# eddyxzc/lpopc

Measured on AMD Instinct MI355X. Metric: eval_g+eval_jac_g calls/sec, 4-phase 4096-LGR-pt problem, higher is better.
Workload: dtype f64

## Files before the change

lpopc_amd/csrc/rpm_abi.cpp:

```cpp
#include <cmath>
#include <cstdio>
#include <cstring>
#include <vector>
#include <new>
#include <string>

#include <atomic>

#include "rpm_engine.hpp"
#include "rpm_pin.h"

static thread_local std::string g_create_error;

using rpm::Engine;

#define RPM_GUARD_BEGIN try {
#define RPM_GUARD_END(eng)                                   \
  }                                                          \
  catch (const std::exception& ex) {                         \
    (eng).err = std::string("internal error: ") + ex.what(); \
    return RPM_E_INVALID;                                    \
  }                                                          \
  catch (...) {                                              \
    (eng).err = "internal error";                            \
// ... 660 lines not shown
      e.role_looped = value == 1 || (value == -1 && total / 64 >= 512);
      rpm::build_tiles(e, e.role_looped ? 64 : 16);
    }
  } else
    return fail(e, RPM_E_INVALID, "unknown option");
  rpm::host_new_x(e);
  rpm::dev_forget_persistent(e);
  return RPM_OK;
}
int rpm_get_option(rpm_engine* h, const char* key, int* value) {
  if (!h || !key || !value) return RPM_E_INVALID;
  Engine& e = h->e;
  const std::string k(key);
  if (k == "fuse_pair") *value = e.opt_fuse_pair;
  else if (k == "check_finite") *value = e.opt_check_finite;
  else if (k == "dx_mode") *value = e.opt_dx_mode;
  else if (k == "tile_nodes") *value = e.tile_nodes;
  else if (k == "n_tiles") *value = int(e.tiles.size());
  else if (k == "role_loop") *value = e.role_looped ? 1 : 0;
  else if (k == "pipeline") *value = e.opt_pipeline;
  else if (k == "mesh_err_tile") *value = e.opt_mesh_err_tile;
  else if (k == "carry_tile") *value = e.opt_carry_tile;
  else if (k == "carry_lds_bytes") *value = e.opt_carry_lds;
  else if (k == "carry_groups") *value = rpm::carry_group_count(e);
  else if (k == "extract_tile") *value = e.opt_extract_tile;
  else if (k == "extract_lds_bytes") *value = e.opt_extract_lds;
  else if (k == "extract_groups") *value = rpm::extract_group_count(e);
  else if (k == "stage_roles") *value = e.opt_stage_roles;
  else if (k == "const_once") *value = e.opt_const_once;
  else if (k == "instance_align") *value = e.opt_instance_align;
  else if (k == "delta_values") *value = e.opt_delta_values;
  else if (k == "ipm_nested") *value = e.opt_ipm_nested;
  else if (k == "ipm_nested_group") *value = e.opt_ipm_nested_group;
  else if (k == "ipm_local_border") *value = e.opt_ipm_local_border;
  else if (k == "zero_copy") *value = e.opt_zero_copy;
  else if (k == "persistent_values") *value = e.opt_persistent_values;
  else if (k == "pin_host") *value = e.opt_pin_host;
  else if (k == "pin_registered") *value = int(rpm::dev_pin_counter(RPM_PIN_REGISTERED));
  else if (k == "pin_register_failures") *value = int(rpm::dev_pin_counter(RPM_PIN_REGISTER_FAILURES));
  else if (k == "pin_unregistered") *value = int(rpm::dev_pin_counter(RPM_PIN_UNREGISTERED));
  else if (k == "pin_unregister_failures") *value = int(rpm::dev_pin_counter(RPM_PIN_UNREGISTER_FAILURES));
  else if (k == "pin_overlap_refused") *value = int(rpm::dev_pin_counter(RPM_PIN_OVERLAP_REFUSED));
  else if (k == "pin_shared") *value = int(rpm::dev_pin_counter(RPM_PIN_SHARED));
  else if (k == "pin_merged") *value = int(rpm::dev_pin_counter(RPM_PIN_MERGED));
  else if (k == "pin_evicted") *value = int(rpm::dev_pin_counter(RPM_PIN_EVICTED));
  else if (k == "pin_live") *value = int(rpm::dev_pin_counter(RPM_PIN_LIVE));
  else if (k == "pin_live_kb") *value = int(rpm::dev_pin_counter(RPM_PIN_LIVE_BYTES) / 1024);
  else if (k == "pin_held") *value = rpm::dev_pin_held(e);
  else if (k == "delta_sent_runs") return rpm::host_delta_sent_runs(e, value);
  else if (k == "delta_total_runs") *value = e.last_delta_total;
  else if (k == "stride_g") *value = int(e.stride_g());
  else if (k == "stride_values") *value = int(e.stride_values());
  else if (k == "pipeline_active") *value = rpm::dev_pipeline_active(e);
  else if (k == "hess_tile_nodes") *value = rpm::dev_hess_tile_nodes(e);
  else return fail(e, RPM_E_INVALID, "unknown option");
  return RPM_OK;
}

int rpm_get_phase_sizes(rpm_engine* h, int phase, int* n_nodes, int* d_nnz, int* doff_nnz) {
  if (!h) return RPM_E_INVALID;
  Engine& e = h->e;
  if (phase < 0 || phase >= e.P) return fail(e, RPM_E_INVALID, "The phase index is out of rang");
  if (n_nodes) *n_nodes = e.ph[phase].N;
  if (d_nnz) *d_nnz = int(e.ph[phase].d_v.size());
  if (doff_nnz) *doff_nnz = int(e.ph[phase].off_v.size());
  return RPM_OK;
}
int rpm_get_phase_tables(rpm_engine* h, int phase, double* points, double* weights, int* d_rows, int* d_cols,
                         double* d_vals, double* diag_vals, int* doff_rows, int* doff_cols, double* doff_vals) {
  if (!h) return RPM_E_INVALID;
  Engine& e = h->e;
  if (phase < 0 || phase >= e.P) return fail(e, RPM_E_INVALID, "The phase index is out of rang");
  const rpm::PhaseHost& p = e.ph[phase];
  auto cp = [](auto* dst, const auto& v) {
    if (dst && !v.empty()) std::memcpy(dst, v.data(), v.size() * sizeof(v[0]));
  };
  cp(points, p.points);
  cp(weights, p.weights);
  cp(d_rows, p.d_i);
  cp(d_cols, p.d_j);
  cp(d_vals, p.d_v);
  cp(diag_vals, p.diag_v);
  cp(doff_rows, p.off_i);
  cp(doff_cols, p.off_j);
  cp(doff_vals, p.off_v);
  return RPM_OK;
}

int rpm_shard_segments(rpm_engine* h, int which, int rank, rpm_segment* seg, int* n_seg, int* packed_len) {
  if (!h) return RPM_E_INVALID;
  Engine& e = h->e;
  RPM_GUARD_BEGIN
  if (which < 0 || which > 1 || rank < 0 || rank >= e.shard_world) return fail(e, RPM_E_INVALID, "shard_segments: bad argument");
  int plen = 0;
  std::vector<rpm_segment> s = rpm::shard_segments(e, which, rank, &plen);
  if (seg) {
    if (!n_seg || *n_seg < int(s.size())) return fail(e, RPM_E_INVALID, "shard_segments: segment buffer too small");
    std::memcpy(seg, s.data(), s.size() * sizeof(rpm_segment));
  }
  if (n_seg) *n_seg = int(s.size());
  if (packed_len) *packed_len = plen;
  return RPM_OK;
  RPM_GUARD_END(e)
}
int rpm_shard_pack_dev(rpm_engine* h, int which, const double* d_full, double* d_packed, void* stream) {
  if (!h) return RPM_E_INVALID;
// ... 35 lines not shown
```

lpopc_amd/csrc/rpm_engine.hpp:

```cpp
#pragma once
#include <cstddef>
#include <string>
#include <utility>
#include <vector>

#include "../../include/rpm_hip.h"

namespace rpm {

struct PhaseDev {
  int N, nx, nu, nc, ne;
  int nq;
  int phase_num;
  int x_state0;
  int x_control0;
  int x_t0;
  int g0;
  int v_nl0;
  int v_evt0;
  int node0;
  int doff_base;
  int off_nnz;
  int const_cum;
  int tile0, ntiles;
// ... 182 lines not shown
             std::string* why);
  int smooth_enough(int ip, int first_row, int n, const std::vector<double>& tau, const double* state, int ld, int nx) const;
  bool exponent(int ip, double m0, double mf, int N, double e_k, double* q) const;
};
void lagrange_rows(const double* src, int m, const double* dst, int nq, double* H, double* S, int* hit);

void build_mesh_err_tables(const PhaseHost& p, MeshErrTables& t);
bool ph_refine(const PhaseHost& p, const double* rel, double tol, int nmin, int nmax, std::vector<double>& mesh,
               std::vector<int>& nodes, std::vector<double>& interval_error);
int dev_solution_error(Engine& e, int phase, const double* x, double* rel_err);
void solution_error_batch_sizes(const Engine& e, int* n_intervals_total, long long* rel_doubles_total);
constexpr double mesh_err_max(double a, double v) { return (v > a || v != v) ? v : a; }
int dev_solution_error_batch(Engine& e, const double* d_x, const int* d_mask, double* d_interval_error, double* d_rel_err_max,
                             double* d_rel_err, int* d_nonfinite, void* stream);
int host_solution_error_batch(Engine& e, const double* x, const int* mask, double* interval_error, double* rel_err_max,
                              double* rel_err, int* nonfinite);

int carry_check(Engine& from, const Engine& to, const void* x_from, const void* x_to);
int carry_group_count(const Engine& from);
int dev_carry_batch(Engine& from, Engine& to, const double* d_x_from, double* d_x_to, int* d_nonfinite, void* stream);
int host_carry_batch(Engine& from, Engine& to, const double* x_from, double* x_to, int* nonfinite);

void nlp2op_batch_layout(const Engine& e, int phase, long long field_offset[8], long long* block_doubles);
int extract_check(Engine& e);
int extract_group_count(const Engine& e);
int dev_nlp2op_batch(Engine& e, const double* d_x, const double* d_lambda, double* d_out, int* d_nonfinite, void* stream);
int host_nlp2op_batch(Engine& e, const double* x, const double* lambda, double* out, int* nonfinite);

std::vector<rpm_segment> shard_segments(const Engine& e, int which, int rank, int* packed_len);
int dev_shard_copy(Engine& e, int which, bool pack, const double* src, int stride, double* dst, void* stream);
long long shard_slot_len(const Engine& e);
int dev_shard_pack_all(Engine& e, const double* d_g, const double* d_values, double* d_slot, void* stream);
int dev_shard_unpack_all(Engine& e, const double* d_gathered, double* d_g, double* d_values, int skip_own, void* stream);

struct ProblemDims { int nx, nu, nc, ne_max, nlink_max, nconst; bool has_analytic; int nq; };
bool problem_dims(int problem_id, ProblemDims* out);

int device_init(Engine& e, int device_id);
void device_destroy(Engine& e);
int dev_eval_cons(Engine& e, const double* d_x, double* d_g, double* d_values, int flags, void* stream);
int dev_eval_obj(Engine& e, const double* d_x, double* d_obj, double* d_grad, void* stream, bool host_chk = false);
bool dev_cons_is_one_role(const Engine& e);
int host_eval_f(Engine& e, const double* x, int new_x, double* obj);
int host_eval_grad_f(Engine& e, const double* x, int new_x, double* grad);
int host_eval_g(Engine& e, const double* x, int new_x, double* g);
void host_new_x(Engine& e);
int host_eval_jac_values(Engine& e, const double* x, int new_x, double* values);
int host_eval_pair(Engine& e, const double* x, double* g, double* values);
struct ConsCall { bool want_g, want_v, cached, delta, launched_jac; };
int host_cons_begin(Engine& e, const double* x, int new_x, double* g, double* values, ConsCall* c);
int host_cons_end(Engine& e, double* g, double* values, const ConsCall& c, const char* who);
int host_delta_sent_runs(Engine& e, int* sent);
int dev_pipeline_active(const Engine& e);
int dev_upload_x(Engine& e, const double* x);
int dev_upload(Engine& e, double* dev, const double* host, size_t count, int slot);
int dev_download(Engine& e, double* host, const double* dev, size_t count, int slot);
int dev_sync(Engine& e);
int dev_update_instance_constants(Engine& e);
double* dev_buf(Engine& e, int which);
bool& dev_cache_valid(Engine& e);
void dev_forget_persistent(Engine& e);
void* dev_stream(Engine& e);
int dev_nonfinite(Engine& e, const double* dev, size_t count);
int dev_nonfinite_enqueue(Engine& e, const double* a, size_t na, const double* b, size_t nb);
int dev_flag_value(Engine& e, int slot);
long dev_pin_counter(int which);
int dev_pin_held(const Engine& e);
void* dev_pin_host(Engine& e, const void* ptr, size_t bytes);
void dev_pin_release_all(Engine& e);

}

struct rpm_engine {
  rpm::Engine e;
};
```

lpopc_amd/csrc/rpm_tile_kernels.hip:

```cpp
#include "rpm_device_internal.hpp"

namespace rpm {


template <class Prob, bool WG, bool WJ, bool AN, bool WAVE = false>
__device__ void endpoint_block(const KParams& K, const TaskDev task, const double* __restrict__ x,
                               double* __restrict__ g, double* __restrict__ vals, double* lds, int inst) {
  constexpr int NX = Prob::NX, NQ = prob_nq<Prob>::value, NQs = NQ > 0 ? NQ : 1;
  bool bad_g = false, bad_j = false;
  constexpr int NE = Prob::NE_MAX > 0 ? Prob::NE_MAX : 1;
  constexpr int NL = Prob::NLINK_MAX > 0 ? Prob::NLINK_MAX : 1;
  static_assert(!WAVE || 2 * NX + 3 + 2 * NQ <= 64, "endpoint perturbations must fit one wave");
  const int tid = WAVE ? int(threadIdx.x & 63) : int(threadIdx.x);
  const int nthr = WAVE ? 64 : int(blockDim.x);
  const double* c = K.consts + size_t(inst) * K.consts_stride;
  if (task.type == 0) {
    for (int r = tid; r < K.P + K.L; r += nthr) {
      if (WG) {
        double acc = 0.0;
        acc += K.alin_v[2 * r] * x[K.alin_j[2 * r]];
        acc += K.alin_v[2 * r + 1] * x[K.alin_j[2 * r + 1]];
        g[K.m_nl + r] = acc;
        chk_note(bad_g, acc);
      }
// ... 508 lines not shown
#pragma unroll
          for (int o = 0; o < NO; ++o) {
            double v0, vf;
            if (o < NX) {
              const double fb = Fb[o * T + kk];
              const double dt = J[o] * (tf - t0) / 2.0;
              v0 = fb * (0.5) - a0 * dt;
              vf = -fb * (0.5) + af * dt;
            } else {
              v0 = a0 * J[o];
              vf = af * J[o];
            }
            vb[size_t(o * NB + NX + NU) * N] = v0;
            vb[size_t(o * NB + NX + NU + 1) * N] = vf;
          }
        }
      }
    }
  }
  RPM_TRC(4);
  if (WJ && !K.skip_const) {
    const double* __restrict__ src = K.doff_vals + tl.c_src0;
    double* __restrict__ dst = vals + tl.c_dst0;
    const int lead = int((reinterpret_cast<size_t>(dst) >> 3) & 15);
    for (int q = tid - lead; q < tl.c_cnt; q += NTHR) {
      if (q >= 0) {
        const double dv = src[q];
#pragma unroll
        for (int i = 0; i < NX; ++i) dst[size_t(i) * tl.c_stride + q] = dv;
      }
    }
  }
#ifdef RPM_DIAG
  RPM_TRC(5);
  if (K.trace) {
    __builtin_amdgcn_s_waitcnt(0);
    RPM_TRC(6);
    if (threadIdx.x == 0) {
      unsigned hw;
      asm volatile("s_getreg_b32 %0, hwreg(HW_REG_HW_ID)" : "=s"(hw));
      unsigned xcc;
      asm volatile("s_getreg_b32 %0, hwreg(HW_REG_XCC_ID)" : "=s"(xcc));
      K.trace[(size_t(blockIdx.y) * gridDim.x + blockIdx.x) * 8 + 7] = (static_cast<unsigned long long>(xcc) << 32) | hw;
    }
  }
#endif
}

constexpr int PL_CMAX = 1280, PL_REC = 32;
static_assert(sizeof(TileDev) / sizeof(int) < PL_REC, "tile record plus the instance index must fit the staged record");
static_assert(sizeof(TileDev) % 8 == 0, "the tile record is copied as doubles");

struct PlLds {
  int rec, next, tt, X, U, D, tau, diag, nodes, cv, stage;
  int Fb, ready, DXs, half;
  __host__ __device__ constexpr PlLds(int nx, int nu, int nc, int nq, int max_span, int max_drow, int max_cshare, bool with_jac,
                                      bool dxm)
      : rec(0), next(PL_REC / 2), tt(PL_REC), X(tt + 2 + ((nq + 1) & ~1)), U(X + nx * max_span), D(U + nu * 64),
        tau(D + max_drow), diag(tau + 64), nodes(diag + 64), cv(nodes + 2 * 64), stage(cv + (with_jac ? max_cshare : 0)),
        Fb(2 * stage), ready(Fb + (nx + nc) * 64), DXs(ready + 2), half(DXs + (dxm ? nx * 64 : 0)) {}
};
constexpr bool pl_lds_pinned(int nx, int nu, int nc, int nq, int span, int drow, int cshare, bool wj, bool dxm) {
  const PlLds L(nx, nu, nc, nq, span, drow, cshare, wj, dxm);
  const int nqe = (nq + 1) & ~1;
  return L.rec == 0 && L.next == L.rec + PL_REC / 2 && L.tt == L.next + PL_REC / 2 && L.X == L.tt + 2 + nqe &&
         L.U == L.X + nx * span && L.D == L.U + nu * 64 && L.tau == L.D + drow && L.diag == L.tau + 64 &&
         L.nodes == L.diag + 64 && L.cv == L.nodes + 2 * 64 && L.stage == L.cv + (wj ? cshare : 0) && L.Fb == 2 * L.stage &&
         L.ready == L.Fb + (nx + nc) * 64 && L.DXs == L.ready + 2 && L.half == L.DXs + (dxm ? nx * 64 : 0) &&
         L.stage == PL_REC + 2 + nqe + nx * span + nu * 64 + drow + 4 * 64 + (wj ? cshare : 0) &&
         L.half == 2 * L.stage + (nx + nc) * 64 + 2 + (dxm ? nx * 64 : 0);
}
static_assert(pl_lds_pinned(LaunchProblem::NX, LaunchProblem::NU, LaunchProblem::NC, 0, 73, 64 * 9, 1024, true, false) &&
                  pl_lds_pinned(LaunchProblem::NX, LaunchProblem::NU, LaunchProblem::NC, 1, 80, 64 * 17, 1280, true, true) &&
                  pl_lds_pinned(QuadrotorProblem::NX, QuadrotorProblem::NU, QuadrotorProblem::NC, 0, 65, 64 * 65, 640, false, true),
              "PlLds: an array overlaps its neighbour or a size changed");
typedef double d2u __attribute__((ext_vector_type(2), aligned(8)));
#define RPM_GPTR(p) ((const __attribute__((address_space(1))) void*)(p))
#define RPM_LPTR(p) ((__attribute__((address_space(3))) void*)(p))
template <int NPART>
__device__ __forceinline__ void pl_dma_run(const double* gsrc, double* ldst, int len, int lane, int part) {
  const int pairs = len >> 1;
#pragma unroll 1
  for (int ch = part; ch * 64 < pairs; ch += NPART)
    if (ch * 64 + lane < pairs)
      __builtin_amdgcn_global_load_lds(RPM_GPTR(gsrc + ch * 128 + 2 * lane), RPM_LPTR(ldst + ch * 128), 16, 0, 0);
  if ((len & 1) && part == 0 && lane < 2)
    __builtin_amdgcn_global_load_lds(RPM_GPTR(reinterpret_cast<const int*>(gsrc + len - 1) + lane),
                                     RPM_LPTR(ldst + len - 1), 4, 0, 0);
}


template <int NX, int NPART>
__device__ __forceinline__ void pl_const_stores(const double* cur, const double* cv_src, int inst_word, double* __restrict__ vall,
                                                long long sv, int lane, int part) {
  constexpr int CCH = (PL_CMAX / 128 + NPART - 1) / NPART;
  const int* rec = reinterpret_cast<const int*>(cur);
  const int c_dst0 = RPM_REC(rec, c_dst0);
  const int inst = __builtin_amdgcn_readfirstlane(rec[inst_word]);
  const int c_cnt = RPM_REC(rec, c_cnt);
  const int c_stride = RPM_REC(rec, c_stride);
  double* __restrict__ cdst = vall + size_t(inst) * sv + c_dst0;
  const int head = min(int((16 - ((reinterpret_cast<size_t>(cdst) >> 3) & 15)) & 15), c_cnt);
  d2u cv[CCH];
#pragma unroll
  for (int ch = 0; ch < CCH; ++ch) {
    const int q = max(min(head + (NPART * ch + part) * 128 + 2 * lane, c_cnt - 2), 0);
    cv[ch].x = cv_src[q];
    cv[ch].y = cv_src[q + 1];
  }
  const bool odd_tail = ((c_cnt - head) & 1) != 0;
  const int edge = lane < head ? lane : (lane == head && odd_tail ? c_cnt - 1 : -1);
  const double cedge = cv_src[max(edge, 0)];
#pragma unroll
  for (int ch = 0; ch < CCH; ++ch) {
    const int q = head + (NPART * ch + part) * 128 + 2 * lane;
    if (q + 1 < c_cnt) {
#pragma unroll
      for (int i = 0; i < NX; ++i) __builtin_nontemporal_store(cv[ch], reinterpret_cast<d2u*>(cdst + size_t(i) * c_stride + q));
    }
  }
  if (part == 0 && edge >= 0) {
#pragma unroll
    for (int i = 0; i < NX; ++i) cdst[size_t(i) * c_stride + edge] = cedge;
  }
}

constexpr int pl_role_groups(int R) { return (R + (R + 11) / 12 - 1) / ((R + 11) / 12); }

struct PlShape { int NH, RG, NDMA; };
constexpr PlShape pl_shape(int R) { return R <= 12 ? PlShape{2, 4, 2} : PlShape{1, pl_role_groups(R), 2}; }

template <class Prob, int NH, int RG, int NDMA, bool WG, bool WJ, bool AN, bool DXM = false, bool STG = false>
__global__ __launch_bounds__(NH * 64 * (RG + NDMA), 1) void rpm_tile_pl_kernel(
    const KParams K, int n_inst, const double* __restrict__ xall, double* __restrict__ gall,
    double* __restrict__ vall) {
  constexpr int T = 64;
  constexpr int HT = 64 * (RG + NDMA);
  constexpr int NX = Prob::NX, NU = Prob::NU, NC = Prob::NC, NQ = prob_nq<Prob>::value;
  constexpr int NXs = NX > 0 ? NX : 1, NUs = NU + NQ > 0 ? NU + NQ : 1;
  constexpr int NO = NX + NC, NV = NX + NU + 1 + NQ, NB = NX + NU + 2 + NQ;
  constexpr int R = WJ ? NV + 1 : (NX > 0 ? NX : 1);
  constexpr int NCs = NC > 0 ? NC : 1;
  constexpr int NTHR = T * RG;
  constexpr int NREC = int(sizeof(TileDev) / sizeof(int));
  extern __shared__ double lds_all[];
  const int half = NH > 1 ? __builtin_amdgcn_readfirstlane(int(threadIdx.x) / HT) : 0;
  const int tid = int(threadIdx.x) - half * HT;
  const int nb = int(gridDim.x), wg = xcd_place(int(blockIdx.x), nb);
  const int G = NH * nb, w = NH * wg + half;
  const int nt = K.n_my_tiles;
  const int W = nt * n_inst;
  const int n_iter = w < W ? (W - w + G - 1) / G : 0;
  const int n_iter_wg = (W - NH * wg + G - 1) / G;
  const PlLds L(NX, NU, NC, NQ, K.max_span, K.max_drow, K.max_cshare, WJ, DXM);
  const int S_TT = L.tt, S_X = L.X, S_U = L.U, S_D = L.D, S_TAU = L.tau, S_DG = L.diag, S_ND = L.nodes, S_CV = L.cv, S_SIZE = L.stage;
  double* lds = lds_all + half * L.half;
  double *Fb = lds + L.Fb, *DXs = lds + L.DXs;
  int* fb_ready = reinterpret_cast<int*>(lds + L.ready);
  int* dx_ready = fb_ready + 1;
#ifdef RPM_DIAG
#define RPM_PTRC(j, slot)                                                           \
  if (K.trace && (threadIdx.x & 63) == 0 && (j) < 2) K.trace[size_t(w) * 64 + (j)*32 + (slot)] = wall_clock64()
#define RPM_PEDGE(slot) \
  if (K.trace && (threadIdx.x & 63) == 0) K.trace[size_t(w) * 64 + (slot)] = wall_clock64()
#define RPM_PEDGE_MAX(slot) \
  if (K.trace && (threadIdx.x & 63) == 0) atomicMax(K.trace + size_t(w) * 64 + (slot), (unsigned long long)wall_clock64())
#else
#define RPM_PTRC(j, slot)
#define RPM_PEDGE(slot)
#define RPM_PEDGE_MAX(slot)
#endif
  if (tid == 0) { RPM_PTRC(0, 31); }

  struct TileRuns { int k0, cnt, span0, span_len, drow0, drow_len, N, x_state0, x_control0, x_t0, node0, c_src0, c_cnt; };
  auto runs_of = [&](auto p) {
    return TileRuns{RPM_REC(p, k0), RPM_REC(p, cnt), RPM_REC(p, span0), RPM_REC(p, span_len), RPM_REC(p, drow0),
                    RPM_REC(p, drow_len), RPM_REC(p, N), RPM_REC(p, x_state0), RPM_REC(p, x_control0), RPM_REC(p, x_t0),
                    RPM_REC(p, node0), RPM_REC(p, c_src0), RPM_REC(p, c_cnt)};
  };
  auto stage = [&](auto np_c, int part, int lane, int item, double* buf, const TileRuns tl) {
    constexpr int NP = decltype(np_c)::value;
    const int inst = item / nt, tidx = item - inst * nt;
    const double* __restrict__ x = xall + size_t(inst) * K.n;
    int rot = 0;
    auto run = [&](const double* gsrc, double* ldst, int len) {
      pl_dma_run<NP>(gsrc, ldst, len, lane, (part + NP - (rot++ % NP)) % NP);
    };
    if (part == 0 && lane == 0) reinterpret_cast<int*>(buf + L.rec)[NREC] = inst;
    run(reinterpret_cast<const double*>(K.tiles + tidx), buf + L.rec, NREC / 2);
    if (item + G < W) {
      const int item2 = item + G, inst2 = item2 / nt;
      run(reinterpret_cast<const double*>(K.tiles + (item2 - inst2 * nt)), buf + L.next, NREC / 2);
    }
    run(x + tl.x_t0, buf + S_TT, 2 + NQ);
#pragma unroll
    for (int i = 0; i < NX; ++i) run(x + tl.x_state0 + i * (tl.N + 1) + tl.span0, buf + S_X + i * K.max_span, tl.span_len);
#pragma unroll
    for (int j = 0; j < NU; ++j) run(x + tl.x_control0 + j * tl.N + tl.k0, buf + S_U + j * T, tl.cnt);
    run(K.points + tl.node0 + tl.k0, buf + S_TAU, tl.cnt);
    if (WJ) run(K.diag + tl.node0 + tl.k0, buf + S_DG, tl.cnt);
    run(reinterpret_cast<const double*>(K.nodes + tl.node0 + tl.k0), buf + S_ND, 2 * tl.cnt);
    if (WG) run(K.dvals + tl.drow0, buf + S_D, tl.drow_len);
    if (WJ && !K.skip_const) run(K.doff_vals + tl.c_src0, buf + S_CV, tl.c_cnt);
  };
  const auto first_runs = [&]() { return runs_of((const __attribute__((address_space(4))) int*)(K.tiles + (w - (w / nt) * nt))); };
  if (tid >= NTHR) {
    const int lane = (tid - NTHR) & 63;
    const int dw = __builtin_amdgcn_readfirstlane((tid - NTHR) >> 6);
    __builtin_amdgcn_s_setprio(3);
    if (dw == 0 && lane == 0) { *fb_ready = 0; *dx_ready = 0; }
    {
      const auto r0 = first_runs();
      RPM_PTRC(0, 19);
      if (n_iter > 0) stage(std::integral_constant<int, NDMA>{}, dw, lane, w, lds, r0);
      RPM_PTRC(0, 20);
    }
#ifdef RPM_DIAG
    unsigned long long wait_sum = 0, wait_max = 0;
#endif
    for (int j = 0; j < n_iter_wg; ++j) {
      const double* cur = lds + (j & 1) * S_SIZE;
      double* nxt = lds + ((j + 1) & 1) * S_SIZE;
#ifdef RPM_DIAG
      const unsigned long long tw0 = wall_clock64();
#endif
      __builtin_amdgcn_s_waitcnt(0);
#ifdef RPM_DIAG
      const unsigned long long tw = wall_clock64() - tw0;
      wait_sum += tw;
      wait_max = tw > wait_max ? tw : wait_max;
#endif
      __syncthreads();
      RPM_PTRC(j, 16);
      if constexpr (DXM && WG) {
        if (j < n_iter) {
          typedef double d4 __attribute__((ext_vector_type(4)));
          const int* rec = reinterpret_cast<const int*>(cur + L.rec);
          const int cnt = RPM_REC(rec, cnt);
          const int span0 = RPM_REC(rec, span0);
          const int drow0 = RPM_REC(rec, drow0);
          const NodeDev* ND = reinterpret_cast<const NodeDev*>(cur + S_ND);
          const double* Ds = cur + S_D;
          const double* Xs = cur + S_X;
          const int lr = lane & 15, kq = lane >> 4;
          for (int rb = 16 * dw; rb < cnt; rb += 16 * NDMA) {
            const int row = rb + lr;
            const bool row_ok = row < cnt;
            const NodeDev ndr = ND[row_ok ? row : cnt - 1];
            const int rel0 = ndr.dcol0 - span0;
            const double* drow = Ds + (ndr.drow_off - drow0);
            const NodeDev nfirst = ND[rb], nlast = ND[min(rb + 15, cnt - 1)];
            const int kmin = __builtin_amdgcn_readfirstlane(nfirst.dcol0 - span0);
            const int kmax = __builtin_amdgcn_readfirstlane(nlast.dcol0 + nlast.dlen - span0);
            for (int cb = 0; cb < NX; cb += 16) {
              const int st = cb + lr;
              d4 acc = {0.0, 0.0, 0.0, 0.0};
              for (int k0 = kmin; k0 < kmax; k0 += 4) {
                const int kcol = k0 + kq;
                const int rel = kcol - rel0;
                const double a = (row_ok && rel >= 0 && rel < ndr.dlen) ? drow[rel] : 0.0;
                const double b = (st < NX && kcol < kmax) ? Xs[st * K.max_span + kcol] : 0.0;
                acc = __builtin_amdgcn_mfma_f64_16x16x4f64(a, b, acc, 0, 0, 0);
              }
#pragma unroll
              for (int i = 0; i < 4; ++i) {
                const int orow = rb + kq + 4 * i;
                if (st < NX && orow < cnt) DXs[st * T + orow] = acc[i];
              }
            }
          }
          if (lane == 0) __hip_atomic_fetch_add(dx_ready, 1, __ATOMIC_RELEASE, __HIP_MEMORY_SCOPE_WORKGROUP);
        }
      }
      if (WJ && !K.skip_const && j < n_iter) pl_const_stores<NX, NDMA>(cur + L.rec, cur + S_CV, NREC, vall, K.sv, lane, dw);
      RPM_PTRC(j, 17);
      if (j + 1 < n_iter) {
        stage(std::integral_constant<int, NDMA>{}, dw, lane, w + (j + 1) * G, nxt, runs_of(reinterpret_cast<const int*>(cur + L.next)));
      }
      RPM_PTRC(j, 18);
    }
#ifdef RPM_DIAG
    if (K.trace && lane == 0 && n_iter > 0) {
      K.trace[size_t(w) * 64 + 28 + dw] = wait_sum;
      K.trace[size_t(w) * 64 + 32 + 28 + dw] = wait_max;
    }
#endif
    const int n_end = K.n_tasks * n_inst;
    for (int it = NDMA * w + dw; it < n_end; it += NDMA * G) {
      const int inst = it / K.n_tasks;
      endpoint_block<Prob, WG, WJ, AN, true>(K, K.tasks[it - inst * K.n_tasks], xall + size_t(inst) * K.n,
                                             gall + size_t(inst) * K.sg, vall + size_t(inst) * K.sv, nullptr, inst);
    }
    return;
  }

  const int kk = tid % T, grp = __builtin_amdgcn_readfirstlane(tid / T);
  for (int jt = 0; jt < n_iter_wg; ++jt) {
    const double* cur = lds + (jt & 1) * S_SIZE;
    asm volatile("s_waitcnt lgkmcnt(0)\n\ts_barrier" ::: "memory");
    if (jt >= n_iter) continue;
    if (grp < 4) { RPM_PTRC(jt, grp * 4 + 0); }
    if (grp == 0 && jt == n_iter - 1) { RPM_PEDGE(22); }
    const int* rec = reinterpret_cast<const int*>(cur + L.rec);
    const int k0 = RPM_REC(rec, k0);
    const int cnt = RPM_REC(rec, cnt);
    const int span0 = RPM_REC(rec, span0);
    const int drow0 = RPM_REC(rec, drow0);
    const int N = RPM_REC(rec, N);
    const int phase_num = RPM_REC(rec, phase_num);
    const int g0 = RPM_REC(rec, g0);
    const int v_nl0 = RPM_REC(rec, v_nl0);
    const int inst = __builtin_amdgcn_readfirstlane(rec[NREC]);
    double* __restrict__ g = gall + size_t(inst) * K.sg;
    double* __restrict__ vals = vall + size_t(inst) * K.sv;
    const auto c4 = (const __attribute__((address_space(4))) double*)(K.consts + size_t(inst) * K.consts_stride);
    const double* Xs = cur + S_X;
    const double* Us = cur + S_U;
    const double* Ds = cur + S_D;
    const int kc = kk < cnt ? kk : cnt - 1;
    const int k = k0 + kc;
    const bool node_ok = kk < cnt;
    bool first = true, no_chk = false;
    typename stage_of<Prob>::type base_stage;
    if constexpr (STG) {
      static_assert(NQ == 0 && !AN, "staged evaluation: finite differences, no static parameters");
      double xs0[NXs], us0[NUs];
#pragma unroll
      for (int i = 0; i < NX; ++i) xs0[i] = Xs[i * K.max_span + (k - span0)];
#pragma unroll
      for (int j = 0; j < NU; ++j) us0[j] = Us[j * T + kc];
      const double tau0 = cur[S_TAU + kc], t00 = cur[S_TT], tf0 = cur[S_TT + 1];
      Prob::stage(phase_num, (tau0 + 1) * ((tf0 - t00) / 2.0) + t00, xs0, us0, c4, base_stage);
    }
// ... 73 lines not shown
          store_defect<T, false>(sv, dx, tf - t0, Fb, kk, g, g0, N, k, no_chk);
        }
        if (WJ && role >= 1) {
          double J[NO];
#pragma unroll
          for (int o = 0; o < NO; ++o) {
            const double pert = o < NX ? f[o < NX ? o : 0] : cp[o >= NX ? o - NX : 0];
            J[o] = AN ? pert : (pert - Fb[o * T + kk]) / h;
          }
          double* __restrict__ vb = vals + v_nl0;
          if (v != NX + NU) {
            const int bv = v < NX + NU ? v : v + 1;
#pragma unroll
            for (int o = 0; o < NO; ++o) {
              double val;
              if (o < NX) {
                const double ret = J[o] * (tf - t0) / 2.0;
                val = (o == v) ? ddiag - ret : -ret;
              } else {
                val = J[o];
              }
              (vb + size_t(o * NB + bv) * N)[k] = val;
            }
          } else {
            const double a0 = -(tau * 0.5) + 0.5, af = (tau * 0.5) + 0.5;
#pragma unroll
            for (int o = 0; o < NO; ++o) {
              double v0, vf;
              if (o < NX) {
                const double fb = Fb[o * T + kk];
                const double dt = J[o] * (tf - t0) / 2.0;
                v0 = fb * (0.5) - a0 * dt;
                vf = -fb * (0.5) + af * dt;
              } else {
                v0 = a0 * J[o];
                vf = af * J[o];
              }
              (vb + size_t(o * NB + NX + NU) * N)[k] = v0;
              (vb + size_t(o * NB + NX + NU + 1) * N)[k] = vf;
            }
          }
        }
      }
#ifdef RPM_DIAG
      if (trc) { RPM_PTRC(jt, 27); }
#endif
    }
    if (grp < 4) { RPM_PTRC(jt, grp * 4 + 3); }
    if (jt == n_iter - 1) { RPM_PEDGE_MAX(23); }
  }
}

static size_t pl_lds_bytes(int nx, int nu, int nc, int nq, const KParams& kp, bool dxm) {
  const PlLds L(nx, nu, nc, nq, kp.max_span, kp.max_drow, kp.max_cshare, true, dxm);
  return size_t(pl_shape(nx + nu + 2 + nq).NH) * L.half * sizeof(double);
}

void tile_pipeline_setup(Engine& e, Device* d, const ProblemDims& pd, int device_id) {
    int ncu = 0;
    if (hipDeviceGetAttribute(&ncu, hipDeviceAttributeMultiprocessorCount, device_id) != hipSuccess || ncu <= 0) ncu = 256;
    const int max_c = d->kp.max_cshare;
    int per_cu = 0;
    with_problem(e.problem_id, [&](auto prob) {
      using P = decltype(prob);
      constexpr PlShape S = pl_shape(P::NX + P::NU + 2 + prob_nq<P>::value);
      d->pl_lds = pl_lds_bytes(pd.nx, pd.nu, pd.nc, pd.nq, d->kp, false);
      if (d->pl_lds > 160 * 1024) return;
      auto kern = rpm_tile_pl_kernel<P, S.NH, S.RG, S.NDMA, true, true, false>;
      if (d->pl_lds > 64 * 1024)
        (void)hipFuncSetAttribute(reinterpret_cast<const void*>(kern), hipFuncAttributeMaxDynamicSharedMemorySize,
                                  int(d->pl_lds));
      if (hipOccupancyMaxActiveBlocksPerMultiprocessor(&per_cu, kern, S.NH * 64 * (S.RG + S.NDMA), d->pl_lds) != hipSuccess)
        per_cu = 0;
      (void)hipGetLastError();
      per_cu *= S.NH;
    });
    d->pl_slots = per_cu * ncu;
    d->pl_ok = e.role_looped && e.tile_nodes == 64 && max_c <= PL_CMAX && max_c >= 2 && 2 * pd.nx + 3 + 2 * pd.nq <= 64 &&
               per_cu >= 1;
}

template <class Kern>
static hipError_t allow_lds(Kern kern, size_t bytes) {
  if (bytes <= 64 * 1024) return hipSuccess;
  return hipFuncSetAttribute(reinterpret_cast<const void*>(kern), hipFuncAttributeMaxDynamicSharedMemorySize, int(bytes));
}

template <class Kern>
static hipError_t launch_tiles(const Engine& e, Kern kern, int threads, const KParams& kp, const double* dx, double* dg,
                               double* dv, hipStream_t st) {
  const Device& d = *e.dev;
  hipError_t s = allow_lds(kern, d.lds_bytes);
  if (s != hipSuccess) return s;
  dim3 grid(unsigned(d.kp.n_my_tiles + d.kp.n_tasks), unsigned(e.n_instances));
  if (grid.x == 0) return hipSuccess;
  hipLaunchKernelGGL(kern, grid, dim3(threads), d.lds_bytes, st, kp, dx, dg, dv);
  return hipGetLastError();
}

static bool pl_dxm_ok(const Engine& e) {
  ProblemDims pd;
  problem_dims(e.problem_id, &pd);
  return e.first_derive != RPM_DERIVE_ANALYTIC && pl_lds_bytes(pd.nx, pd.nu, pd.nc, pd.nq, e.dev->kp, true) <= 160 * 1024;
}

template <class Prob, bool WG, bool WJ, bool AN, bool DXM, bool STG = false>
static hipError_t launch_tile_pl(const Engine& e, const KParams& kp, const double* dx, double* dg, double* dv, hipStream_t st) {
  if constexpr (!STG && !AN && has_stage<Prob>::value) {
    if (e.opt_stage_roles == 1 || (e.opt_stage_roles < 0 && (kp.skip_const || stage_always<Prob>::value)))
      return launch_tile_pl<Prob, WG, WJ, AN, DXM, true>(e, kp, dx, dg, dv, st);
  }
  const Device& d = *e.dev;
  constexpr PlShape S = pl_shape(Prob::NX + Prob::NU + 2 + prob_nq<Prob>::value);
  auto kern = rpm_tile_pl_kernel<Prob, S.NH, S.RG, S.NDMA, WG, WJ, AN, DXM, STG>;
  const size_t lds = pl_lds_bytes(Prob::NX, Prob::NU, Prob::NC, prob_nq<Prob>::value, d.kp, DXM);
  hipError_t s = allow_lds(kern, lds);
  if (s != hipSuccess) return s;
  const long long W = (long long)d.kp.n_my_tiles * e.n_instances;
  const long long halves = W < d.pl_slots ? W : d.pl_slots;
  hipLaunchKernelGGL(kern, dim3(unsigned((halves + S.NH - 1) / S.NH)), dim3(S.NH * 64 * (S.RG + S.NDMA)), lds, st, kp,
                     e.n_instances, dx, dg, dv);
  return hipGetLastError();
}

static bool use_pipeline(const Engine& e) {
  const Device& d = *e.dev;
  if (!d.pl_ok || e.opt_pipeline == 0 || d.kp.n_my_tiles <= 0) return false;
  if (e.opt_pipeline == 1) return true;
  const long long W = (long long)d.kp.n_my_tiles * e.n_instances;
  return W >= 2LL * d.pl_slots || (W <= d.pl_slots && 4 * W >= 3LL * d.pl_slots);
}

static int cons_layout(const Engine& e) {
  if (!(e.role_looped && e.tile_nodes == 64)) return 0;
  if (e.opt_dx_mode == 0) return use_pipeline(e) ? 2 : 1;
  return (use_pipeline(e) && pl_dxm_ok(e)) ? 2 : 0;
}
bool dev_cons_is_one_role(const Engine& e) { return !e.dev || cons_layout(e) == 0; }

int dev_pipeline_active(const Engine& e) { return e.dev && cons_layout(e) == 2 ? 1 : 0; }

template <bool WG_, bool WJ_, bool AN_, bool DXM_>
struct TileFlags { static constexpr bool WG = WG_, WJ = WJ_, AN = AN_, DXM = DXM_; };

template <class Prob, class Launch>
static hipError_t with_tile_flags(const Engine& e, bool wg, bool wj, Launch&& launch) {
  if constexpr (Prob::HAS_ANALYTIC) {
    if (wj && e.first_derive == RPM_DERIVE_ANALYTIC)
      return wg ? launch(TileFlags<true, true, true, false>{}) : launch(TileFlags<false, true, true, false>{});
  }
  if (wg && e.opt_dx_mode == 1)
    return wj ? launch(TileFlags<true, true, false, true>{}) : launch(TileFlags<true, false, false, true>{});
  if (wg && wj) return launch(TileFlags<true, true, false, false>{});
  if (wj) return launch(TileFlags<false, true, false, false>{});
  return launch(TileFlags<true, false, false, false>{});
}

template <class Prob, int T>
static hipError_t launch_tile_T(const Engine& e, const KParams& kp, bool wg, bool wj, const double* dx, double* dg,
                                double* dv, hipStream_t st) {
  const int layout = T == 64 ? cons_layout(e) : 0;
  return with_tile_flags<Prob>(e, wg, wj, [&](auto flags) -> hipError_t {
    using F = decltype(flags);
    if constexpr (T == 64) {
      if (layout == 2) return launch_tile_pl<Prob, F::WG, F::WJ, F::AN, F::DXM>(e, kp, dx, dg, dv, st);
      if constexpr (!F::DXM) {
        if (layout == 1) return launch_tiles(e, rpm_tile_rl_kernel<Prob, 64, 4, F::WG, F::WJ, F::AN>, 64 * 4, kp, dx, dg, dv, st);
      }
    }
    constexpr int R = F::WJ ? Prob::NX + Prob::NU + 2 + prob_nq<Prob>::value : (Prob::NX > 0 ? Prob::NX : 1);
    constexpr int threads = (T * R + 63) / 64 * 64;
    return launch_tiles(e, rpm_tile_kernel<Prob, T, F::WG, F::WJ, F::AN, F::DXM>, threads, kp, dx, dg, dv, st);
  });
}

int dev_eval_cons(Engine& e, const double* d_x, double* d_g, double* d_values, int flags, void* stream) {
  if (!e.dev) {
    int rc = device_init(e, 0);
    if (rc) return rc;
  }
  hipStream_t st = static_cast<hipStream_t>(stream);
  const bool wg = flags & 1, wj = flags & 2;
  KParams kp = e.dev->kp;
  kp.sg = (flags & 4) ? e.stride_g() : e.m;
  kp.sv = (flags & 4) ? e.stride_values() : e.nnz_jac;
  kp.chk = ((flags & 8) && dev_cons_is_one_role(e)) ? e.dev->d_flags2 : nullptr;
  kp.skip_const = 0;
  if (wj && (flags & 16) && d_values) {
    auto& seen = e.dev->const_filled;
    if (std::find(seen.begin(), seen.end(), d_values) != seen.end()) {
      kp.skip_const = 1;
    } else {
      if (seen.size() >= 4096) seen.clear();
// ... 21 lines not shown
```

Baseline: 632,200.

## Keep shared constant Jacobian values in DMA-wave registers instead of LDS staging

The DMA waves of the pipelined tile kernel no longer stage each tile's constant off-diagonal Jacobian values through LDS. Each wave now holds them in registers (PlShare) and reloads only when the tile's values or alignment head change; when the grid stride is a multiple of the tile count, a wave revisits the same tile, so the load happens once. This removes the cv LDS region, shrinking LDS per half, and cuts repeated global reads of doff_vals. The wait/barrier structure is also reworked: a raw s_barrier with a partial waitcnt replaces __syncthreads, and a full wait moves to the end of the iteration. This adds register pressure and a new introspection option.

After: 625,600. 1.0% lower.

```diff
diff --git a/lpopc_amd/csrc/rpm_abi.cpp b/lpopc_amd/csrc/rpm_abi.cpp
--- a/lpopc_amd/csrc/rpm_abi.cpp
+++ b/lpopc_amd/csrc/rpm_abi.cpp
@@ -736,6 +736,7 @@
   else if (k == "stride_g") *value = int(e.stride_g());
   else if (k == "stride_values") *value = int(e.stride_values());
   else if (k == "pipeline_active") *value = rpm::dev_pipeline_active(e);
+  else if (k == "pipeline_share_once") *value = rpm::dev_pipeline_share_once(e);
   else if (k == "hess_tile_nodes") *value = rpm::dev_hess_tile_nodes(e);
   else return fail(e, RPM_E_INVALID, "unknown option");
   return RPM_OK;
diff --git a/lpopc_amd/csrc/rpm_engine.hpp b/lpopc_amd/csrc/rpm_engine.hpp
--- a/lpopc_amd/csrc/rpm_engine.hpp
+++ b/lpopc_amd/csrc/rpm_engine.hpp
@@ -258,6 +258,7 @@
 int host_cons_end(Engine& e, double* g, double* values, const ConsCall& c, const char* who);
 int host_delta_sent_runs(Engine& e, int* sent);
 int dev_pipeline_active(const Engine& e);
+int dev_pipeline_share_once(const Engine& e);
 int dev_upload_x(Engine& e, const double* x);
 int dev_upload(Engine& e, double* dev, const double* host, size_t count, int slot);
 int dev_download(Engine& e, double* host, const double* dev, size_t count, int slot);
diff --git a/lpopc_amd/csrc/rpm_tile_kernels.hip b/lpopc_amd/csrc/rpm_tile_kernels.hip
--- a/lpopc_amd/csrc/rpm_tile_kernels.hip
+++ b/lpopc_amd/csrc/rpm_tile_kernels.hip
@@ -584,27 +584,26 @@
 static_assert(sizeof(TileDev) % 8 == 0, "the tile record is copied as doubles");
 
 struct PlLds {
-  int rec, next, tt, X, U, D, tau, diag, nodes, cv, stage;
+  int rec, next, tt, X, U, D, tau, diag, nodes, stage;
   int Fb, ready, DXs, half;
-  __host__ __device__ constexpr PlLds(int nx, int nu, int nc, int nq, int max_span, int max_drow, int max_cshare, bool with_jac,
-                                      bool dxm)
+  __host__ __device__ constexpr PlLds(int nx, int nu, int nc, int nq, int max_span, int max_drow, bool dxm)
       : rec(0), next(PL_REC / 2), tt(PL_REC), X(tt + 2 + ((nq + 1) & ~1)), U(X + nx * max_span), D(U + nu * 64),
-        tau(D + max_drow), diag(tau + 64), nodes(diag + 64), cv(nodes + 2 * 64), stage(cv + (with_jac ? max_cshare : 0)),
+        tau(D + max_drow), diag(tau + 64), nodes(diag + 64), stage(nodes + 2 * 64),
         Fb(2 * stage), ready(Fb + (nx + nc) * 64), DXs(ready + 2), half(DXs + (dxm ? nx * 64 : 0)) {}
 };
-constexpr bool pl_lds_pinned(int nx, int nu, int nc, int nq, int span, int drow, int cshare, bool wj, bool dxm) {
-  const PlLds L(nx, nu, nc, nq, span, drow, cshare, wj, dxm);
+constexpr bool pl_lds_pinned(int nx, int nu, int nc, int nq, int span, int drow, bool dxm) {
+  const PlLds L(nx, nu, nc, nq, span, drow, dxm);
   const int nqe = (nq + 1) & ~1;
   return L.rec == 0 && L.next == L.rec + PL_REC / 2 && L.tt == L.next + PL_REC / 2 && L.X == L.tt + 2 + nqe &&
          L.U == L.X + nx * span && L.D == L.U + nu * 64 && L.tau == L.D + drow && L.diag == L.tau + 64 &&
-         L.nodes == L.diag + 64 && L.cv == L.nodes + 2 * 64 && L.stage == L.cv + (wj ? cshare : 0) && L.Fb == 2 * L.stage &&
+         L.nodes == L.diag + 64 && L.stage == L.nodes + 2 * 64 && L.Fb == 2 * L.stage &&
          L.ready == L.Fb + (nx + nc) * 64 && L.DXs == L.ready + 2 && L.half == L.DXs + (dxm ? nx * 64 : 0) &&
-         L.stage == PL_REC + 2 + nqe + nx * span + nu * 64 + drow + 4 * 64 + (wj ? cshare : 0) &&
+         L.stage == PL_REC + 2 + nqe + nx * span + nu * 64 + drow + 4 * 64 &&
          L.half == 2 * L.stage + (nx + nc) * 64 + 2 + (dxm ? nx * 64 : 0);
 }
-static_assert(pl_lds_pinned(LaunchProblem::NX, LaunchProblem::NU, LaunchProblem::NC, 0, 73, 64 * 9, 1024, true, false) &&
-                  pl_lds_pinned(LaunchProblem::NX, LaunchProblem::NU, LaunchProblem::NC, 1, 80, 64 * 17, 1280, true, true) &&
-                  pl_lds_pinned(QuadrotorProblem::NX, QuadrotorProblem::NU, QuadrotorProblem::NC, 0, 65, 64 * 65, 640, false, true),
+static_assert(pl_lds_pinned(LaunchProblem::NX, LaunchProblem::NU, LaunchProblem::NC, 0, 73, 64 * 9, false) &&
+                  pl_lds_pinned(LaunchProblem::NX, LaunchProblem::NU, LaunchProblem::NC, 1, 80, 64 * 17, true) &&
+                  pl_lds_pinned(QuadrotorProblem::NX, QuadrotorProblem::NU, QuadrotorProblem::NC, 0, 65, 64 * 65, true),
               "PlLds: an array overlaps its neighbour or a size changed");
 typedef double d2u __attribute__((ext_vector_type(2), aligned(8)));
 #define RPM_GPTR(p) ((const __attribute__((address_space(1))) void*)(p))
@@ -622,38 +621,55 @@
 }
 
 
+template <int NPART>
+struct PlShare {
+  static constexpr int CCH = (PL_CMAX / 128 + NPART - 1) / NPART;
+  static constexpr int NLOADS = CCH + 1;
+  d2u cv[CCH];
+  double cedge;
+  int head;
+};
+__device__ __forceinline__ int pl_share_head(const double* cdst, int c_cnt) {
+  return min(int((16 - ((reinterpret_cast<size_t>(cdst) >> 3) & 15)) & 15), c_cnt);
+}
+__device__ __forceinline__ int pl_share_edge(int head, int c_cnt, int lane) {
+  const bool odd_tail = ((c_cnt - head) & 1) != 0;
+  return lane < head ? lane : (lane == head && odd_tail ? c_cnt - 1 : -1);
+}
+template <int NPART>
+__device__ __forceinline__ void pl_share_load(PlShare<NPART>& S, const double* doff_vals, int c_src0, int c_cnt, int head,
+                                              int lane, int part) {
+  const double* pairs = doff_vals + (c_cnt >= 2 ? c_src0 : 0);
+#pragma unroll
+  for (int ch = 0; ch < PlShare<NPART>::CCH; ++ch) {
+    const int q = max(min(head + (NPART * ch + part) * 128 + 2 * lane, c_cnt - 2), 0);
+    S.cv[ch] = *reinterpret_cast<const d2u*>(pairs + q);
+  }
+  S.cedge = (doff_vals + (c_cnt >= 1 ? c_src0 : 0))[max(pl_share_edge(head, c_cnt, lane), 0)];
+  S.head = head;
+}
 template <int NX, int NPART>
-__device__ __forceinline__ void pl_const_stores(const double* cur, const double* cv_src, int inst_word, double* __restrict__ vall,
+__device__ __forceinline__ void pl_const_stores(const double* cur, const PlShare<NPART>& S, int inst_word, double* __restrict__ vall,
                                                 long long sv, int lane, int part) {
-  constexpr int CCH = (PL_CMAX / 128 + NPART - 1) / NPART;
   const int* rec = reinterpret_cast<const int*>(cur);
   const int c_dst0 = RPM_REC(rec, c_dst0);
   const int inst = __builtin_amdgcn_readfirstlane(rec[inst_word]);
   const int c_cnt = RPM_REC(rec, c_cnt);
   const int c_stride = RPM_REC(rec, c_stride);
   double* __restrict__ cdst = vall + size_t(inst) * sv + c_dst0;
-  const int head = min(int((16 - ((reinterpret_cast<size_t>(cdst) >> 3) & 15)) & 15), c_cnt);
-  d2u cv[CCH];
-#pragma unroll
-  for (int ch = 0; ch < CCH; ++ch) {
-    const int q = max(min(head + (NPART * ch + part) * 128 + 2 * lane, c_cnt - 2), 0);
-    cv[ch].x = cv_src[q];
-    cv[ch].y = cv_src[q + 1];
-  }
-  const bool odd_tail = ((c_cnt - head) & 1) != 0;
-  const int edge = lane < head ? lane : (lane == head && odd_tail ? c_cnt - 1 : -1);
-  const double cedge = cv_src[max(edge, 0)];
-#pragma unroll
-  for (int ch = 0; ch < CCH; ++ch) {
+  const int head = S.head;
+#pragma unroll
+  for (int ch = 0; ch < PlShare<NPART>::CCH; ++ch) {
     const int q = head + (NPART * ch + part) * 128 + 2 * lane;
     if (q + 1 < c_cnt) {
 #pragma unroll
-      for (int i = 0; i < NX; ++i) __builtin_nontemporal_store(cv[ch], reinterpret_cast<d2u*>(cdst + size_t(i) * c_stride + q));
-    }
-  }
+      for (int i = 0; i < NX; ++i) __builtin_nontemporal_store(S.cv[ch], reinterpret_cast<d2u*>(cdst + size_t(i) * c_stride + q));
+    }
+  }
+  const int edge = pl_share_edge(head, c_cnt, lane);
   if (part == 0 && edge >= 0) {
 #pragma unroll
-    for (int i = 0; i < NX; ++i) cdst[size_t(i) * c_stride + edge] = cedge;
+    for (int i = 0; i < NX; ++i) cdst[size_t(i) * c_stride + edge] = S.cedge;
   }
 }
 
@@ -684,8 +700,8 @@
   const int W = nt * n_inst;
   const int n_iter = w < W ? (W - w + G - 1) / G : 0;
   const int n_iter_wg = (W - NH * wg + G - 1) / G;
-  const PlLds L(NX, NU, NC, NQ, K.max_span, K.max_drow, K.max_cshare, WJ, DXM);
-  const int S_TT = L.tt, S_X = L.X, S_U = L.U, S_D = L.D, S_TAU = L.tau, S_DG = L.diag, S_ND = L.nodes, S_CV = L.cv, S_SIZE = L.stage;
+  const PlLds L(NX, NU, NC, NQ, K.max_span, K.max_drow, DXM);
+  const int S_TT = L.tt, S_X = L.X, S_U = L.U, S_D = L.D, S_TAU = L.tau, S_DG = L.diag, S_ND = L.nodes, S_SIZE = L.stage;
   double* lds = lds_all + half * L.half;
   double *Fb = lds + L.Fb, *DXs = lds + L.DXs;
   int* fb_ready = reinterpret_cast<int*>(lds + L.ready);
@@ -704,11 +720,11 @@
 #endif
   if (tid == 0) { RPM_PTRC(0, 31); }
 
-  struct TileRuns { int k0, cnt, span0, span_len, drow0, drow_len, N, x_state0, x_control0, x_t0, node0, c_src0, c_cnt; };
+  struct TileRuns { int k0, cnt, span0, span_len, drow0, drow_len, N, x_state0, x_control0, x_t0, node0, c_src0, c_cnt, c_dst0; };
   auto runs_of = [&](auto p) {
     return TileRuns{RPM_REC(p, k0), RPM_REC(p, cnt), RPM_REC(p, span0), RPM_REC(p, span_len), RPM_REC(p, drow0),
                     RPM_REC(p, drow_len), RPM_REC(p, N), RPM_REC(p, x_state0), RPM_REC(p, x_control0), RPM_REC(p, x_t0),
-                    RPM_REC(p, node0), RPM_REC(p, c_src0), RPM_REC(p, c_cnt)};
+                    RPM_REC(p, node0), RPM_REC(p, c_src0), RPM_REC(p, c_cnt), RPM_REC(p, c_dst0)};
   };
   auto stage = [&](auto np_c, int part, int lane, int item, double* buf, const TileRuns tl) {
     constexpr int NP = decltype(np_c)::value;
@@ -733,7 +749,6 @@
     if (WJ) run(K.diag + tl.node0 + tl.k0, buf + S_DG, tl.cnt);
     run(reinterpret_cast<const double*>(K.nodes + tl.node0 + tl.k0), buf + S_ND, 2 * tl.cnt);
     if (WG) run(K.dvals + tl.drow0, buf + S_D, tl.drow_len);
-    if (WJ && !K.skip_const) run(K.doff_vals + tl.c_src0, buf + S_CV, tl.c_cnt);
   };
   const auto first_runs = [&]() { return runs_of((const __attribute__((address_space(4))) int*)(K.tiles + (w - (w / nt) * nt))); };
   if (tid >= NTHR) {
@@ -741,28 +756,58 @@
     const int dw = __builtin_amdgcn_readfirstlane((tid - NTHR) >> 6);
     __builtin_amdgcn_s_setprio(3);
     if (dw == 0 && lane == 0) { *fb_ready = 0; *dx_ready = 0; }
+    using Share = PlShare<NDMA>;
+    Share share;
+    const bool has_share = WJ && !K.skip_const && n_iter > 0;
+    const bool share_once = G % nt == 0;
+    auto share_head = [&](int item, int c_dst0, int c_cnt) { return pl_share_head(vall + size_t(item / nt) * K.sv + c_dst0, c_cnt); };
+#ifdef RPM_DIAG
+    unsigned long long wait_sum = 0, wait_max = 0;
+    unsigned long long tw0;
+#define RPM_PWAIT_BEGIN tw0 = wall_clock64()
+#define RPM_PWAIT_END                                \
+  {                                                  \
+    const unsigned long long tw = wall_clock64() - tw0; \
+    wait_sum += tw;                                  \
+    wait_max = tw > wait_max ? tw : wait_max;        \
+  }
+    unsigned long long t19 = 0, t20 = 0;
+#else
+#define RPM_PWAIT_BEGIN
+#define RPM_PWAIT_END
+#endif
     {
       const auto r0 = first_runs();
-      RPM_PTRC(0, 19);
+#ifdef RPM_DIAG
+      t19 = wall_clock64();
+#endif
       if (n_iter > 0) stage(std::integral_constant<int, NDMA>{}, dw, lane, w, lds, r0);
-      RPM_PTRC(0, 20);
-    }
 #ifdef RPM_DIAG
-    unsigned long long wait_sum = 0, wait_max = 0;
+      t20 = wall_clock64();
 #endif
+      if (has_share) {
+        asm volatile("" ::: "memory");
+        pl_share_load(share, K.doff_vals, r0.c_src0, r0.c_cnt, share_head(w, r0.c_dst0, r0.c_cnt), lane, dw);
+        RPM_PWAIT_BEGIN;
+        asm volatile("s_waitcnt vmcnt(%0) lgkmcnt(0)" ::"n"(Share::NLOADS) : "memory");
+        RPM_PWAIT_END;
+      } else {
+        RPM_PWAIT_BEGIN;
+        __builtin_amdgcn_s_waitcnt(0);
+        RPM_PWAIT_END;
+      }
+    }
     for (int j = 0; j < n_iter_wg; ++j) {
       const double* cur = lds + (j & 1) * S_SIZE;
       double* nxt = lds + ((j + 1) & 1) * S_SIZE;
+      asm volatile("s_barrier" ::: "memory");
+      __builtin_amdgcn_s_waitcnt(0x0F70);
 #ifdef RPM_DIAG
-      const unsigned long long tw0 = wall_clock64();
+      if (j == 0 && K.trace && lane == 0) {
+        K.trace[size_t(w) * 64 + 19] = t19;
+        K.trace[size_t(w) * 64 + 20] = t20;
+      }
 #endif
-      __builtin_amdgcn_s_waitcnt(0);
-#ifdef RPM_DIAG
-      const unsigned long long tw = wall_clock64() - tw0;
-      wait_sum += tw;
-      wait_max = tw > wait_max ? tw : wait_max;
-#endif
-      __syncthreads();
       RPM_PTRC(j, 16);
       if constexpr (DXM && WG) {
         if (j < n_iter) {
@@ -804,13 +849,25 @@
           if (lane == 0) __hip_atomic_fetch_add(dx_ready, 1, __ATOMIC_RELEASE, __HIP_MEMORY_SCOPE_WORKGROUP);
         }
       }
-      if (WJ && !K.skip_const && j < n_iter) pl_const_stores<NX, NDMA>(cur + L.rec, cur + S_CV, NREC, vall, K.sv, lane, dw);
+      if (has_share && j < n_iter) pl_const_stores<NX, NDMA>(cur + L.rec, share, NREC, vall, K.sv, lane, dw);
       RPM_PTRC(j, 17);
       if (j + 1 < n_iter) {
-        stage(std::integral_constant<int, NDMA>{}, dw, lane, w + (j + 1) * G, nxt, runs_of(reinterpret_cast<const int*>(cur + L.next)));
+        const TileRuns r1 = runs_of(reinterpret_cast<const int*>(cur + L.next));
+        if (has_share) {
+          const int head = share_head(w + (j + 1) * G, r1.c_dst0, r1.c_cnt);
+          if (!share_once || head != share.head) pl_share_load(share, K.doff_vals, r1.c_src0, r1.c_cnt, head, lane, dw);
+        }
+        stage(std::integral_constant<int, NDMA>{}, dw, lane, w + (j + 1) * G, nxt, r1);
       }
       RPM_PTRC(j, 18);
-    }
+      if (j + 1 < n_iter_wg) {
+        RPM_PWAIT_BEGIN;
+        __builtin_amdgcn_s_waitcnt(0);
+        RPM_PWAIT_END;
+      }
+    }
+#undef RPM_PWAIT_BEGIN
+#undef RPM_PWAIT_END
 #ifdef RPM_DIAG
     if (K.trace && lane == 0 && n_iter > 0) {
       K.trace[size_t(w) * 64 + 28 + dw] = wait_sum;
@@ -990,7 +1047,7 @@
 }
 
 static size_t pl_lds_bytes(int nx, int nu, int nc, int nq, const KParams& kp, bool dxm) {
-  const PlLds L(nx, nu, nc, nq, kp.max_span, kp.max_drow, kp.max_cshare, true, dxm);
+  const PlLds L(nx, nu, nc, nq, kp.max_span, kp.max_drow, dxm);
   return size_t(pl_shape(nx + nu + 2 + nq).NH) * L.half * sizeof(double);
 }
 
@@ -1042,6 +1099,13 @@
   return e.first_derive != RPM_DERIVE_ANALYTIC && pl_lds_bytes(pd.nx, pd.nu, pd.nc, pd.nq, e.dev->kp, true) <= 160 * 1024;
 }
 
+static unsigned pl_grid(const Engine& e, int NH) {
+  const Device& d = *e.dev;
+  const long long W = (long long)d.kp.n_my_tiles * e.n_instances;
+  const long long halves = W < d.pl_slots ? W : d.pl_slots;
+  return unsigned((halves + NH - 1) / NH);
+}
+
 template <class Prob, bool WG, bool WJ, bool AN, bool DXM, bool STG = false>
 static hipError_t launch_tile_pl(const Engine& e, const KParams& kp, const double* dx, double* dg, double* dv, hipStream_t st) {
   if constexpr (!STG && !AN && has_stage<Prob>::value) {
@@ -1054,10 +1118,7 @@
   const size_t lds = pl_lds_bytes(Prob::NX, Prob::NU, Prob::NC, prob_nq<Prob>::value, d.kp, DXM);
   hipError_t s = allow_lds(kern, lds);
   if (s != hipSuccess) return s;
-  const long long W = (long long)d.kp.n_my_tiles * e.n_instances;
-  const long long halves = W < d.pl_slots ? W : d.pl_slots;
-  hipLaunchKernelGGL(kern, dim3(unsigned((halves + S.NH - 1) / S.NH)), dim3(S.NH * 64 * (S.RG + S.NDMA)), lds, st, kp,
-                     e.n_instances, dx, dg, dv);
+  hipLaunchKernelGGL(kern, dim3(pl_grid(e, S.NH)), dim3(S.NH * 64 * (S.RG + S.NDMA)), lds, st, kp, e.n_instances, dx, dg, dv);
   return hipGetLastError();
 }
 
@@ -1077,6 +1138,17 @@
 bool dev_cons_is_one_role(const Engine& e) { return !e.dev || cons_layout(e) == 0; }
 
 int dev_pipeline_active(const Engine& e) { return e.dev && cons_layout(e) == 2 ? 1 : 0; }
+
+int dev_pipeline_share_once(const Engine& e) {
+  if (!dev_pipeline_active(e)) return 0;
+  int once = 0;
+  with_problem(e.problem_id, [&](auto prob) {
+    using P = decltype(prob);
+    constexpr PlShape S = pl_shape(P::NX + P::NU + 2 + prob_nq<P>::value);
+    once = (S.NH * (long long)pl_grid(e, S.NH)) % e.dev->kp.n_my_tiles == 0 ? 1 : 0;
+  });
+  return once;
+}
 
 template <bool WG_, bool WJ_, bool AN_, bool DXM_>
 struct TileFlags { static constexpr bool WG = WG_, WJ = WJ_, AN = AN_, DXM = DXM_; };
```
